# Corleno/Nonstationary_Multivariate_Gaussian_Process

Hardware: AMD Instinct MI355X
Metric: log-posterior evals/sec (N=2048, D=3 nonseparable GP) (higher is better)
Workload: dtype f64

## Files before the change

### nonstationary_multivariate_gaussian_process_amd/csrc/nmgp_api.hip

```cpp
#include <cstdarg>

#include "nmgp_internal.h"

using namespace nmgpk;

enum {
    SC_LOGDET = 0,
    SC_QUAD = 1,
    SC_PRIORQ = 2,
    SC_TRACE = 40,
    SC_OUT = 48,
    SC_MISC = 56,
    SC_COUNT = 128
};

int nmgp_fail(nmgp_ctx* ctx, int code, const char* fmt, ...) {
    char buf[1024];
    va_list ap;
    va_start(ap, fmt);
    vsnprintf(buf, sizeof(buf), fmt, ap);
    va_end(ap);
    if (ctx) ctx->err = buf;
    return code;
}
// ... 122 lines not shown
    c->priors.clear();
}

static void free_subject(nmgp_ctx* c) {
    double** ptrs[] = {&c->d_x, &c->d_Y, &c->d_y, &c->d_pars, &c->d_grad, &c->d_ell, &c->d_sig, &c->d_Lv,
                       &c->d_S, &c->d_Sinv, &c->d_z, &c->d_alpha, &c->d_R, &c->d_R2, &c->d_part, &c->d_K, &c->d_K2,
                       &c->d_w, &c->d_E};
    for (double** p : ptrs) {
        if (*p) hipFree(*p);
        *p = nullptr;
    }
    c->S_cap = c->K_cap = c->part_cap = 0;
    if (c->had_indx) hipFree(c->had_indx);
    if (c->had_y) hipFree(c->had_y);
    c->had_indx = nullptr;
    c->had_y = nullptr;
    c->had = false;
    if (c->ps_buf) hipFree(c->ps_buf);
    c->ps_buf = nullptr;
    c->ps_cap = 0;
    free_priors(c);
    {
        double** bp[] = {&c->b_pars, &c->b_ell, &c->b_Lv, &c->b_S, &c->b_z, &c->b_R, &c->b_scal, &c->b_q,
                         &c->b_S2, &c->b_Sinv, &c->b_alpha, &c->b_part, &c->b_grad, &c->b_R2, &c->b_tr, &c->b_u, &c->b_schur};
        c->b_grad_ready = false;
        c->b_multi = false;
        if (c->b_x) hipFree(c->b_x);
        if (c->b_y) hipFree(c->b_y);
        c->b_x = c->b_y = nullptr;
        for (auto& pf : c->b_priors) {
            if (pf.L) hipFree(pf.L);
            if (pf.logdet) hipFree(pf.logdet);
        }
        c->b_priors.clear();
        for (double** p : bp) {
            if (*p) hipFree(*p);
            *p = nullptr;
        }
        if (c->b_info) hipFree(c->b_info);
        if (c->b_info2) hipFree(c->b_info2);
        c->b_info = c->b_info2 = nullptr;
        c->b_schur_stride = 0;
        c->batch = 0;
    }
}

extern "C" int nmgp_version(void) { return NMGP_VERSION; }

extern "C" int nmgp_device_count(void) {
    int n = 0;
    if (hipGetDeviceCount(&n) != hipSuccess) return 0;
    return n;
}

extern "C" int nmgp_ctx_create(int device, nmgp_ctx** out) {
    if (!out) return NMGP_E_NULL;
    *out = nullptr;
    int ndev = 0;
    if (hipGetDeviceCount(&ndev) != hipSuccess || ndev <= 0) return NMGP_E_HIP;
    if (device < 0 || device >= ndev) return NMGP_E_SHAPE;
    nmgp_ctx* c = new nmgp_ctx();
    c->device = device;
    *out = c;
    if (const char* e = std::getenv("NMGP_CHOL")) c->chol_algo = (std::strcmp(e, "rocsolver") == 0) ? 0 : 1;
    if (const char* e = std::getenv("NMGP_CHOL_NB1")) {
        int v = std::atoi(e);
        if (v >= 64) c->chol_nb1 = (v / 64) * 64;
    }
    HIP_TRY(c, hipSetDevice(device));
    if (const char* e = std::getenv("NMGP_CHOL_LOOKAHEAD")) c->chol_lookahead = std::atoi(e);
    if (const char* e = std::getenv("NMGP_PRIOR_SOLVE")) {
        c->prior_rocblas = std::strcmp(e, "rocblas") == 0;
        c->prior_trsv_all = std::strcmp(e, "trsv") == 0;
    }
    if (const char* e = std::getenv("NMGP_SEP")) c->sep_algo = (std::strcmp(e, "eig") == 0) ? 0 : 1;
    if (const char* e = std::getenv("NMGP_SVC_SCHUR")) c->svc_schur = std::atoi(e) != 0 ? 1 : 0;
    {
        int lo = 0, hi = 0;
        hipDeviceGetStreamPriorityRange(&lo, &hi);
        const bool prio = lo != hi;
        if (prio) HIP_TRY(c, hipStreamCreateWithPriority(&c->stream, hipStreamNonBlocking, hi));
        else HIP_TRY(c, hipStreamCreateWithFlags(&c->stream, hipStreamNonBlocking));
        int la_cus = 64;
        if (const char* e = std::getenv("NMGP_LOOKAHEAD_CUS")) la_cus = std::atoi(e);
        hipDeviceProp_t prop{};
        int ncu = 0;
        if (hipGetDeviceProperties(&prop, device) == hipSuccess) ncu = prop.multiProcessorCount;
        const bool mi355 = std::strncmp(prop.gcnArchName, "gfx950", 6) == 0 && ncu == 256;
        if (mi355 && la_cus > 0 && la_cus < ncu) {
            std::vector<uint32_t> mask((size_t)(ncu + 31) / 32, 0u);
            for (int i = la_cus; i < ncu; ++i) mask[(size_t)i / 32] |= 1u << (i % 32);
            if (hipExtStreamCreateWithCUMask(&c->stream2, (uint32_t)mask.size(), mask.data()) != hipSuccess) {
                (void)hipGetLastError();
                c->stream2 = nullptr;
            } else {
                c->stream2_cus = ncu - la_cus;
            }
        }
        if (!c->stream2) {
// ... 402 lines not shown
                               double* grad) {
    if (!c) return NMGP_E_NULL;
    if (!out5) return nmgp_fail(c, NMGP_E_NULL, "out5 must not be NULL");
    NMGP_TRY(nmgp_svc_set_pars(c, pars));
    NMGP_TRY(svc_enqueue(c, hyper, prior, grad != nullptr));
    return nmgp_svc_fetch(c, out5, grad);
}

static void mass_reset(nmgp_ctx* c) {
    double** ptrs[] = {&c->b_minv, &c->b_vel, &c->b_mchol, &c->b_mU, &c->b_mw, &c->b_mc};
    for (double** p : ptrs) {
        if (*p) hipFree(*p);
        *p = nullptr;
    }
    c->b_mass_kind = 0;
    c->b_mrank = 0;
    c->b_traj_ready = false;
}

static void free_batch(nmgp_ctx* c) {
    double** ptrs[] = {&c->b_pars, &c->b_ell, &c->b_Lv, &c->b_S, &c->b_z, &c->b_R, &c->b_scal, &c->b_q,
                       &c->b_S2, &c->b_Sinv, &c->b_alpha, &c->b_part, &c->b_grad, &c->b_R2, &c->b_tr,
                       &c->b_mom, &c->b_q0, &c->b_g0, &c->b_am, &c->b_av, &c->b_minv, &c->b_vel, &c->b_mchol, &c->b_kin,
                       &c->b_mU, &c->b_mw, &c->b_mc, &c->b_u, &c->b_schur};
    c->b_schur_stride = 0;
    c->b_mass_kind = 0;
    c->b_mrank = 0;
    c->b_cps = 1;
    if (c->b_alive) hipFree(c->b_alive);
    c->b_alive = nullptr;
    c->b_adam_t = -1;
    c->b_grad_ready = false;
    c->b_traj_ready = false;
    if (c->b_hmc) hipFree(c->b_hmc);
    c->b_hmc = nullptr;
    c->b_multi = false;
    if (c->b_x) hipFree(c->b_x);
    if (c->b_y) hipFree(c->b_y);
    c->b_x = c->b_y = nullptr;
    for (auto& pf : c->b_priors) {
        if (pf.L) hipFree(pf.L);
        if (pf.logdet) hipFree(pf.logdet);
    }
    c->b_priors.clear();
    for (double** p : ptrs) {
        if (*p) hipFree(*p);
        *p = nullptr;
    }
// ... 132 lines not shown
    }
    c->b_priors.push_back(pf);
    *out = &c->b_priors.back();
    return 0;
}

static int batch_grad_alloc(nmgp_ctx* c) {
    if (c->b_grad_ready) return 0;
    const size_t N = c->N, T = c->T, n = c->n, P = (size_t)c->P_svc, B = c->batch;
    const size_t ld2 = nmgp_ld(2 * n + 2);
    const size_t NJ = (N + 63) / 64;
    NMGP_TRY(nmgp_dev_alloc(c, &c->b_S2, B * ld2 * n));
    NMGP_TRY(nmgp_dev_alloc(c, &c->b_Sinv, B * n * n));
    NMGP_TRY(nmgp_dev_alloc(c, &c->b_alpha, B * n));
    NMGP_TRY(nmgp_dev_alloc(c, &c->b_part, B * std::max(NJ * N * (T + 1), (size_t)n * ((n + 255) / 256))));
    NMGP_TRY(nmgp_dev_alloc(c, &c->b_grad, B * P));
    NMGP_TRY(nmgp_dev_alloc(c, &c->b_R2, N * B * (1 + T)));
    NMGP_TRY(nmgp_dev_alloc(c, &c->b_tr, B * 2));
    c->b_grad_ready = true;
    return 0;
}

static bool schur_selected(const nmgp_ctx* c, int want_grad) {
    if (want_grad || c->M < 2 || c->svc_schur == 0) return false;
    return true;
}

static int svc_batch_value_schur(nmgp_ctx* c, const double* xs, int xstride, const double* ys, long long ystride, int cps) {
    const int N = c->N, M = c->M, B = c->batch, n1 = (M - 1) * N;
    const long long P = c->P_svc;
    const int xpad = (N + 1) & 1, xoffA = N + 1 + xpad;
    const int ldA = (int)nmgp_ld((size_t)2 * N + 2), ldP = (int)nmgp_ld((size_t)n1 + 1);
    auto r64 = [](size_t v) { return (v + 63) / 64 * 64; };
    const size_t offP = r64((size_t)ldA * N), offPart = r64(offP + (size_t)ldP * n1);
    const size_t need = r64(offPart + (size_t)N * ((N + 255) / 256));
    const size_t bsS = nmgp_ld((size_t)c->n + 1) * (size_t)c->n;
    double* base = c->b_S;
    size_t bsz = bsS;
    if (need > bsS) {
        if (c->b_schur_stride != need) {
            NMGP_TRY(nmgp_dev_alloc(c, &c->b_schur, (size_t)B * need));
            c->b_schur_stride = need;
        }
        base = c->b_schur;
        bsz = need;
    }
    const long long bs = (long long)bsz;
// ... 23 lines not shown
    {
        StageScope sp(c, NMGP_STAGE_REDUCE);
        chol_logdet_quad(s, A, ldA, N, w, c->b_scal + 2, c->b_scal + 3, B, bs, 16);
    }
    {
        StageScope sp(c, NMGP_STAGE_INVERSE);
        const SchurEpi e{xs, c->b_ell, c->b_Lv, tse, ys, c->b_u, Sp, ldP, N, xstride, cps, ystride, bs};
        int r = syrk_schur(s, A + xoffA, ldA, N, M, B, e);
        if (r) return nmgp_fail(c, r, "unsupported number of outputs M=%d", M);
    }
    {
        StageScope sp(c, NMGP_STAGE_CHOL);
        nmgp_potrf(c, Sp, ldP, n1, 1, 0, c->b_info2, B, bs, 1);
    }
    {
        StageScope sp(c, NMGP_STAGE_SOLVE);
        get_row(s, Sp, ldP, n1, w1, n1, B, bs, n1);
    }
    {
        StageScope sp(c, NMGP_STAGE_REDUCE);
        chol_logdet_quad(s, Sp, ldP, n1, w1, c->b_scal + 4, c->b_scal + 5, B, bs, 16);
        svc_schur_combine(s, c->b_Lv, N, M, c->b_scal, 16, c->b_info, c->b_info2, B);
    }
    return 0;
}

extern "C" int nmgp_svc_batch_eval(nmgp_ctx* c, const double hyper[8], int prior, int want_grad) {
    if (!c) return NMGP_E_NULL;
    if (!hyper) return nmgp_fail(c, NMGP_E_NULL, "hyper must not be NULL");
    if (c->batch <= 0) return nmgp_fail(c, NMGP_E_STATE, "nmgp_svc_batch_alloc must be called first");
    HIP_TRY(c, hipSetDevice(c->device));
    const int N = c->N, M = c->M, T = c->T, n = c->n, B = c->batch;
    const long long P = c->P_svc;
    c->b_traj_ready = false;
    if (want_grad) NMGP_TRY(batch_grad_alloc(c));
    const int xpad = (n + 1) & 1, xoff = n + 1 + xpad;
    const int ld = want_grad ? (int)nmgp_ld((size_t)2 * n + 2) : (int)nmgp_ld((size_t)n + 1);
    double* S = want_grad ? c->b_S2 : c->b_S;
    const long long bs = (long long)ld * n;
    const double mu_l = hyper[0], al_l = hyper[1], be_l = hyper[2], mu_L = hyper[3], al_L = hyper[4], be_L = hyper[5];
    const double a = hyper[6], b = hyper[7];
    hipStream_t s = c->stream;
    const bool multi = c->b_multi;
    const int cps = multi ? c->b_cps : 1;
    const double* xs = multi ? c->b_x : c->d_x;
    const int xstride = multi ? N : 0;
    PriorFactor *pl = nullptr, *pL = nullptr;
    if (multi) {
        NMGP_TRY(get_batch_prior(c, al_l, be_l, &pl));
        NMGP_TRY(get_batch_prior(c, al_L, be_L, &pL));
        NMGP_TRY(get_batch_prior(c, al_l, be_l, &pl));
    } else {
        NMGP_TRY(nmgp_get_prior(c, al_l, be_l, &pl));
        NMGP_TRY(nmgp_get_prior(c, al_L, be_L, &pL));
        NMGP_TRY(nmgp_get_prior(c, al_l, be_l, &pl));
    }
    HIP_TRY(c, hipMemsetAsync(c->b_info, 0, (size_t)B * sizeof(int), s));
    if (nmgp_poison()) HIP_TRY(c, hipMemsetAsync(c->b_scal, 0xFF, (size_t)B * 16 * sizeof(double), s));
    PriorStreamScope ps(c);
    if (schur_selected(c, want_grad)) {
        NMGP_TRY(svc_batch_value_schur(c, xs, xstride, multi ? c->b_y : c->d_y, multi ? n : 0, cps));
    } else {
        {
            StageScope sp(c, NMGP_STAGE_COV);
            svc_prep(s, c->b_pars, N, M, c->b_ell, c->b_Lv, B);
            int r = svc_cov_build(s, xs, c->b_ell, c->b_Lv, c->b_pars + (P - 1), S, ld, N, M, false, B, bs, xstride, cps);
            if (r) return nmgp_fail(c, r, "unsupported number of outputs M=%d", M);
        }
        {
            StageScope sp(c, NMGP_STAGE_CHOL);
            set_row(s, S, ld, n, multi ? c->b_y : c->d_y, n, B, bs, multi ? n : 0, cps);
            if (want_grad) identity_rows(s, S, ld, n + 1, n, xpad, B, bs);
            nmgp_potrf(c, S, ld, n, want_grad ? 1 + xpad : 1, want_grad ? n : 0, c->b_info, B, bs, 1);
        }
        {
            StageScope sp(c, NMGP_STAGE_SOLVE);
            get_row(s, S, ld, n, c->b_z, n, B, bs, n);
            if (want_grad) {
                tri_gemv_upper(s, S + xoff, (int)ld, n, c->b_z, c->b_alpha, c->b_part, (int)B, bs,
                               (long long)n * ((n + 255) / 256));
            }
        }
        {
// ... 53 lines not shown
                                          B * (1 + T), &one, pl->L, pl->ld, R, N));
            } else {
                const rocblas_stride sB = (rocblas_stride)(1 + T) * N;
                BLAS_TRY(c, rocblas_dtrsm_strided_batched(ps.hb, rocblas_side_left, rocblas_fill_lower, op,
                                                          rocblas_diagonal_non_unit, N, 1, &one, pl->L, pl->ld, 0, R, N, sB, B));
                BLAS_TRY(c, rocblas_dtrsm_strided_batched(ps.hb, rocblas_side_left, rocblas_fill_lower, op,
                                                          rocblas_diagonal_non_unit, N, T, &one, pL->L, pL->ld, 0, R + N, N, sB,
                                                          B));
            }
            if (pass == 0) col_sumsq(ps.sp, c->b_R, N, N, B * (1 + T), c->b_q);
        }
    }
    ps.done();
    ps.join();
    {
        StageScope sp(c, NMGP_STAGE_REDUCE);
        const double ig_const = a * std::log(b) - std::lgamma(a);
        svc_finalize(s, c->b_scal, c->b_scal + 1, c->b_q, pl->logdet, pL->logdet, c->b_pars, P, N, T, a, b, ig_const,
                     prior, c->b_scal + 8, B, 16, multi ? 1 : 0, cps);
    }
    if (want_grad) {
        {
            StageScope sp(c, NMGP_STAGE_INVERSE);
            syrk_lower(s, S + xoff, ld, c->b_Sinv, n, n, n, n, B, bs, (long long)n * n, 2);
        }
        {
            StageScope sp(c, NMGP_STAGE_ADJOINT);
            trace_terms(s, c->b_alpha, c->b_Sinv, n, n, c->b_tr, -1.0, B);
            int r = svc_adjoint(s, xs, c->b_ell, c->b_Lv, c->b_alpha, c->b_Sinv, n, N, M, c->b_part, -1.0, B, xstride, cps);
            if (r) return nmgp_fail(c, r, "unsupported number of outputs M=%d", M);
            svc_grad_final(s, c->b_part, (N + 63) / 64, N, M, c->b_Lv, c->b_R2, N, c->b_pars, c->b_tr, a, b, prior,
                           c->b_grad, B);
        }
    }
    c->b_last_grad = want_grad != 0;
    c->last_kind = 2;
    return nmgp_take_launch_error(c);
}

extern "C" double* nmgp_svc_batch_grad_dev(nmgp_ctx* c) { return c ? c->b_grad : nullptr; }

extern "C" int nmgp_svc_batch_fetch_grad(nmgp_ctx* c, double* grad) {
    if (!c) return NMGP_E_NULL;
    if (!grad) return nmgp_fail(c, NMGP_E_NULL, "grad must not be NULL");
    if (c->last_kind != 2 || !c->b_last_grad)
        return nmgp_fail(c, NMGP_E_STATE, "the last batched evaluation did not compute gradients");
    HIP_TRY(c, hipSetDevice(c->device));
// ... 717 lines not shown
```

### nonstationary_multivariate_gaussian_process_amd/csrc/nmgp_chol.hip

```cpp
#include "nmgp_internal.h"
#include <cstring>

namespace nmgpk {

static inline int cdiv_c(long long a, long long b) { return (int)((a + b - 1) / b); }

typedef double v4d __attribute__((ext_vector_type(4)));

#define SY_BM 128
#define SY_BK 16
#define SY_LD (SY_BM + 16)
#define SY_SB 8

__device__ __forceinline__ int clamp_row_pair(int r, int rows) {
    int rc = r < rows - 1 ? r : rows - 2;
    return rc < 0 ? 0 : rc;
}

__device__ __forceinline__ double fast_recip(double p) {
    double x = __builtin_amdgcn_rcp(p);
    double e = fma(-p, x, 1.0);
    x = fma(x, e, x);
    e = fma(-p, x, 1.0);
    x = fma(x, e, x);
// ... 160 lines not shown
            const double* __restrict__ Lr = e.Lv + (size_t)r * T_;
            const double xr = e.x[r], lr = e.ell[r];
            const double xr2 = xr * xr, lr2 = lr * lr;
            const double l00 = Lr[0];
            const double il2 = 1.0 / (l00 * l00);
#pragma unroll QU
            for (int q = 0; q < 16; ++q) {
                const int o = 2 * q + hi;
                const int il = pass == 0 ? lo : o, jl = pass == 0 ? o : lo;
                const int c = (pass == 0 ? j0 : i0) + o;
                if (pass == 0 ? (c > r || c >= N) : (c <= r || c >= N)) continue;
                const double* gc = gt + (pass == 0 ? c - col0 : 128 + c - row0) * GS;
                if (pass == 1 && M == 3) {
                    e.S[(size_t)c * e.ld + (Ns + r)] = P[il * 33 + jl];
                    continue;
                }
                const double xc = M <= 4 ? gc[M] : e.x[c], lc = M <= 4 ? gc[M + 1] : e.ell[c];
                const double dist = (xr2 + xc * xc) - 2.0 * (xr * xc);
                const double Aa = lr2 + lc * lc;
                double kv = sqrt(2.0 * (lr * lc) / Aa) * exp(-dist / Aa);
                if (r == c) kv = NMGP_JITTER + kv;
                const double nai = P[il * 33 + jl];
                if (pass == 0) {
                    svc_schur_entries<M, true>(e, sigma2, r, Lr, il2, c, kv, nai, gc);
                    if (M == 3 && c < r) {
                        const double* Lc = e.Lv + (size_t)c * T_;
                        P[il * 33 + jl] = svc_schur_value<M>(sigma2, 2, 1, false, Lc, gc[M - 1], Lr, kv, nai, gt[(128 + r - row0) * GS]);
                    }
                } else {
                    svc_schur_entries<M, false>(e, sigma2, r, Lr, il2, c, kv, nai, gc);
                }
            }
        }
        __builtin_amdgcn_wave_barrier();
    }
}

template <int M>
__device__ __forceinline__ void svc_schur_yrow(const SchurEpi& e, int i) {
    constexpr int T = M * (M + 1) / 2;
    if (i >= e.N) return;
    const size_t Ns = (size_t)e.N;
    const int n1 = (M - 1) * e.N;
    const double sigma2 = exp(e.tse[0]);
    const double* Li = e.Lv + (size_t)i * T;
    const double l00 = Li[0];
// ... 298 lines not shown
            bj = c0 + in / rb;
            bi = base + in % rb;
        }
        }
    }
    if (bi < bj) return;
    bi = __builtin_amdgcn_readfirstlane(bi);
    bj = __builtin_amdgcn_readfirstlane(bj);
    bz = __builtin_amdgcn_readfirstlane(bz);
    A += (size_t)bz * bstride;
    C += (size_t)bz * cstride;
    SchurEpi se{};
    if constexpr (SM > 0) {
        static_assert(NWJ == 4 && BK == 16, "the Schur epilogue assumes 8 waves of 64 x 32");
        constexpr int T = SM * (SM + 1) / 2;
        se = *sep;
        se.x += (size_t)(bz / se.cps) * se.xstride;
        se.y += (size_t)(bz / se.cps) * se.ystride;
        se.ell += (size_t)bz * se.N;
        se.Lv += (size_t)bz * se.N * T;
        se.tse += (size_t)bz * ((size_t)se.N * (1 + T) + 1);
        se.u += (size_t)bz * se.N;
        se.S += (size_t)bz * se.bstride;
    }
    const bool diag = (bi == bj);
    const int tid = threadIdx.x, lane = tid & 63, w = tid >> 6;
    const int wi = w & 1, wj = w >> 1;
    const int row0 = bi * SY_BM, col0 = bj * SY_BM;
    if constexpr (NWJ == 4 && BK == 16) {
        const int ncw = ncols - col0 >= SY_BM ? SY_BM : ncols - col0;
        if (row0 + SY_BM <= mrows && (ncw == SY_BM || ncw == 64) && col0 + SY_BM <= mrows && (K & 31) == 0 &&
            (long long)(K + 16) * lda * 8 < 0x7fff0000LL) {
            int kt0f = ktri ? row0 / BK : 0;
            if (row0 >= tri_row0) {
                const int z = (row0 - tri_row0 - tri_k0) / BK;
                kt0f = z > 0 ? (z & ~1) : 0;
            }
            syrk_tile_fast<SM>(A, lda, C, ldc, K, row0, col0, diag, kt0f, ktri != 0, ncw, yrow, nyr, &sA[0][0], &sB[0][0],
                               skipq && bi == 0 && bj == 0, (finfo != nullptr && bi == 0 && bj == 0) ? finfo + (size_t)bz * fistride : nullptr,
                               fgoff, mirror, fresh0, &se);
            return;
        }
    }
    const int rp = tid & 63, cg = tid >> 6;
    double2 ra[NQ], rb[NQ];

// ... 1404 lines not shown
```

### nonstationary_multivariate_gaussian_process_amd/csrc/nmgp_internal.h

```cpp
#pragma once

#include <hip/hip_runtime.h>
#include <rocblas/rocblas.h>
#include <rocsolver/rocsolver.h>

#include <cmath>
#include <cstdio>
#include <cstdlib>
#include <cstring>
#include <map>
#include <string>
#include <utility>
#include <vector>

#include "nmgp.h"

#define NMGP_JITTER 1e-6
#define NMGP_PRECISION 1e-6

struct DevBuf {
    double* p = nullptr;
    size_t cap = 0;
};

// ... 13 lines not shown
    double bytes = 0;
};

struct SyrkHook {
    void* user = nullptr;
    void* (*begin)(void* user, hipStream_t s, double flop, double bytes) = nullptr;
    void (*end)(void* user, void* token) = nullptr;
};

struct nmgp_ctx {
    int device = 0;
    hipStream_t stream = nullptr;
    hipStream_t stream2 = nullptr;
    int stream2_cus = 0;
    hipStream_t stream_prior = nullptr;
    rocblas_handle blas_prior = nullptr;
    hipEvent_t ev_prior_fork = nullptr, ev_prior_join = nullptr;
    int prior_overlap = 1;
    std::vector<hipEvent_t> chol_ev;
    int chol_lookahead = 1;
    SyrkHook syrk_hook;
    int sep_algo = 1;
    int svc_schur = -1;
    rocblas_handle blas = nullptr;
    std::string err;

    int N = 0, M = 0, T = 0, n = 0;
    double* d_x = nullptr;
    double* d_Y = nullptr;
    double* d_y = nullptr;
    bool had = false;
    int* had_indx = nullptr;
    double* had_y = nullptr;
    long long P_svc = 0;
    double* d_pars = nullptr;
    double* d_grad = nullptr;
    double* d_ell = nullptr;
    double* d_sig = nullptr;
    double* d_Lv = nullptr;
    double* d_S = nullptr;
    double* d_Sinv = nullptr;
    size_t S_cap = 0;
    int ldS = 0;
    double* d_z = nullptr;
    double* d_alpha = nullptr;
    double* d_R = nullptr;
// ... 5 lines not shown
    double* h_pin = nullptr;
    int* h_info = nullptr;
    DevBuf scratch[16];
    std::vector<PriorFactor> priors;
    double* d_K = nullptr;
    double* d_K2 = nullptr;
    size_t K_cap = 0;
    double* d_w = nullptr;
    double* d_E = nullptr;
    int batch = 0;
    double* b_pars = nullptr;
    double* b_ell = nullptr;
    double* b_Lv = nullptr;
    double* b_S = nullptr;
    double* b_z = nullptr;
    double* b_R = nullptr;
    double* b_scal = nullptr;
    double* b_q = nullptr;
    int* b_info = nullptr;
    double* b_u = nullptr;
    int* b_info2 = nullptr;
    double* b_schur = nullptr;
    size_t b_schur_stride = 0;
    bool b_grad_ready = false;
    double* b_S2 = nullptr;
    double* b_Sinv = nullptr;
    double* b_alpha = nullptr;
    double* b_part = nullptr;
    double* b_grad = nullptr;
    double* b_R2 = nullptr;
    double* b_tr = nullptr;
    bool b_last_grad = false;
    double* b_mom = nullptr;
    double* b_q0 = nullptr;
    double* b_g0 = nullptr;
    int* b_hmc = nullptr;
    bool b_traj_ready = false;
    double* b_am = nullptr;
    double* b_av = nullptr;
    int* b_alive = nullptr;
    long long b_adam_t = -1;
    bool b_multi = false;
    double* b_x = nullptr;
    double* b_y = nullptr;
    std::vector<PriorFactor> b_priors;
    int b_cps = 1;
// ... 174 lines not shown
               double b1, double b2, double bc2s, double eps, double step, long long P, int B);
void hmc_status(hipStream_t s, const int* info, const double* scal, int* bad, int* failed, int B);
void hmc_kick_drift(hipStream_t s, double* p, const double* g, double* q, const int* bad, double c, double eps, int drift,
                    long long P, int B);
void hmc_drift(hipStream_t s, double* q, const double* p, const double* vel, const double* minv_diag, double eps, long long P, int B);
void hmc_scale(hipStream_t s, double* p, const double* d, long long P, int B);
void hmc_kinetic(hipStream_t s, const double* p, const double* vel, const double* minv_diag, double* kin, long long P, int B);
void hmc_restore(hipStream_t s, double* q, double* g, const double* q0, const double* g0, int* bad, const int* bad0,
                 const int* accept, long long P, int B);
void prior_trmm(hipStream_t s, bool trans, const double* L0, int ld0, long long s0, const double* L1, int ld1, long long s1,
                const double* in, double* out, int N, int T, long long P, int B, int cps, double coef, int mode, const int* bad);
void prior_trmm_sep(hipStream_t s, bool trans, const double* L0, int ld0, const double* L1, int ld1, const double* in, double* out, int N,
                    int T, long long P, int B, double cscale);
void lowrank_proj(hipStream_t s, const double* U, const double* u, double* c, long long P, int r, int B, int cps);
void lowrank_apply(hipStream_t s, const double* U, const double* wgt, const double* c, const double* in, double* out, long long P,
                   int r, int B, int cps);
void metric_kinetic(hipStream_t s, const double* u, const double* c, const double* sw, double* kin, long long P, int r, int B, int cps);
int svc_adjoint(hipStream_t s, const double* x, const double* ell, const double* Lv, const double* alpha,
                const double* Sinv, int ld, int N, int M, double* part, double ssign = 1.0, int batch = 1,
                int xstride = 0, int cps = 1);
#define NMGP_XTRI_SEED_BLOCKS 3
#define NMGP_TRI_GEMV_BLOCK 256
void tri_gemv_upper(hipStream_t s, const double* W, int ld, int n, const double* z, double* out, double* part, int batch = 1,
                    long long wstride = 0, long long pstride = 0);
void trace_terms(hipStream_t s, const double* alpha, const double* Sinv, int ld, int n, double* out,
                 double ssign = 1.0, int batch = 1);
void svc_grad_final(hipStream_t s, const double* part, int NJ, int N, int M, const double* Lv, const double* R2,
                    int ldR, const double* pars, const double* tr, double a, double b, int prior, double* grad,
                    int batch = 1);
void svc_finalize(hipStream_t s, const double* logdet, const double* quad, const double* q, const double* hl_l,
                  const double* hl_L, const double* pars, long long P, int N, int T, double a, double b,
                  double ig_const, int prior, double* out5, int batch = 1, int sstride = 0, int hstride = 0, int cps = 1);
void half_logdet(hipStream_t s, const double* L, int ld, int n, double* out, int batch = 1);
int kron_mv(hipStream_t s, const double* K, int n1, int n2, const double* y, const double* B, int m1, int m2,
            double* out);
void eig_reduce(hipStream_t s, double* a, const double* wB, int M, const double* wK, int N, const double* sigma2p,
                bool scale, double* out);
void colscale_d(hipStream_t s, const double* V, const double* wB, int M, const double* wK, int N, const double* sigma2p,
                double* Vs);
void colscale(hipStream_t s, const double* V, const double* svec, int rows, int cols, double* Vs);
void sep_coreB(hipStream_t s, const double* At, const double* wB, int M, const double* wK, int N,
               const double* sigma2p, double* coreB);
void sep_adjoint(hipStream_t s, const double* x, const double* ell, const double* sig, const double* U,
                 const double* wB, int M, const double* C, int N, double* part);
void sep_grad_sum(hipStream_t s, const double* part, int NJ, int N, double* g);
void exp_vec(hipStream_t s, const double* in, int n, double* out);
void fill_vec(hipStream_t s, double* out, int n, double v);
// ... 38 lines not shown
                   int small_per, int M, const double* C, int N, double* part, double* g, int B);
void two_col_rhs_b(hipStream_t s, const double* pars, long long P, double mu_a, double mu_b, int N, double* R, int B);
void ps_rows_reduce(hipStream_t s, const double* A, int ld, long long bstride, int n, int R0, int zrow, int E, double* part,
                    int batch, double* dots, double* sqs, long long ostride, long long o0);
void pss_star(hipStream_t s, const double* W0, const double* W1, const double* cv0, const double* cv1, const double* pars, long long P,
              const double* z, int N, int S, double mu_l, double mu_s, double* star, int B);
bool syrk_lower(hipStream_t s, const double* A, int lda, double* C, int ldc, int mrows, int ncols, int K, int batch,
                long long bstride, long long cstride = -1, int ktri = 0, int tri_row0 = 0x7fffffff, int tri_k0 = 0,
                int* finfo = nullptr, int fistride = 0, int goff = 0, const SyrkHook* hook = nullptr);
struct SchurEpi {
    const double* x;
    const double* ell;
    const double* Lv;
    const double* tse;
    const double* y;
    const double* u;
    double* S;
    int ld;
    int N;
    int xstride;
    int cps;
    long long ystride;
    long long bstride;
};
int syrk_schur(hipStream_t s, const double* X, int lda, int N, int M, int batch, const SchurEpi& e);
void identity_rows(hipStream_t s, double* A, int lda, int row0, int n, int pad, int batch = 1, long long bstride = 0);
void set_row(hipStream_t s, double* A, int lda, int row, const double* v, int n, int batch, long long bstride,
             long long vstride, int cps = 1);
void get_row(hipStream_t s, const double* A, int lda, int row, double* v, int n, int batch, long long bstride,
             long long vstride);
void potrf_lower(hipStream_t s, hipStream_t s2, hipEvent_t* ev, double* A, int lda, int n, int extra, int xtri,
                 int nb1, int* info, int batch, long long bstride, int istride, const SyrkHook* hook = nullptr,
                 int precise = 0);

}
```

### nonstationary_multivariate_gaussian_process_amd/csrc/nmgp_kernels.hip

```cpp
#include "nmgp_internal.h"
#include <mutex>

namespace nmgpk {

static inline int cdiv(long long a, long long b) { return (int)((a + b - 1) / b); }

__device__ inline double wave_sum(double v) {
#pragma unroll
    for (int off = 32; off > 0; off >>= 1) v += __shfl_down(v, off, 64);
    return v;
}

__device__ inline double block_sum(double v, double* sh ) {
    int lane = threadIdx.x & 63, w = threadIdx.x >> 6;
    v = wave_sum(v);
    __syncthreads();
    if (lane == 0) sh[w] = v;
    __syncthreads();
    int nw = (blockDim.x + 63) >> 6;
    v = (threadIdx.x < nw) ? sh[threadIdx.x] : 0.0;
    if (w == 0) v = wave_sum(v);
    return v;
}

// ... 223 lines not shown
        default: return NMGP_E_UNSUPPORTED;
    }
    return 0;
}

__global__ __launch_bounds__(256) void k_svc_schur_combine(const double* __restrict__ Lv, int N, int T, double* __restrict__ sc,
                                                            int sstride, int* __restrict__ info, const int* __restrict__ info2) {
    __shared__ double sh[16];
    Lv += (size_t)blockIdx.x * N * T;
    sc += (size_t)blockIdx.x * sstride;
    double a = 0.0;
    for (int i = threadIdx.x; i < N; i += blockDim.x) a += log(Lv[(size_t)i * T]);
    a = block_sum(a, sh);
    if (threadIdx.x == 0) {
        sc[0] = (2.0 * a + sc[2]) + sc[4];
        sc[1] = sc[3] + sc[5];
        if (info[blockIdx.x] == 0 && info2[blockIdx.x] != 0) info[blockIdx.x] = N + info2[blockIdx.x];
    }
}

void svc_schur_combine(hipStream_t s, const double* Lv, int N, int M, double* sc, int sstride, int* info, const int* info2,
                       int batch) {
    NMGP_LAUNCH(k_svc_schur_combine, dim3(batch), dim3(256), 0, s, Lv, N, M * (M + 1) / 2, sc, sstride, info, info2);
}

template <bool GIBBS, bool FULL>
__global__ __launch_bounds__(256) void k_cov_sym(const double* __restrict__ x, const double* __restrict__ sig,
                                                  const double* __restrict__ ell, int N, double alpha, double beta,
                                                  double* __restrict__ out, int ld) {
    constexpr int TJ = 64;
    __shared__ double sx[TJ], sl[TJ], ss[TJ];
    const int I = blockIdx.x, J = blockIdx.y;
    if (!FULL && I < J) return;
    x += (size_t)blockIdx.z * N;
    out += (size_t)blockIdx.z * ld * N;
    const int tid = threadIdx.x, lane = tid & 63, w = tid >> 6;
    const int j0 = J * TJ;
    if (tid < TJ) {
        int j = j0 + tid;
        double xv = (j < N) ? x[j] : 0.0;
        sx[tid] = GIBBS ? xv : xv / beta;
        sl[tid] = (GIBBS && j < N) ? ell[j] : 1.0;
        ss[tid] = (GIBBS && sig != nullptr && j < N) ? sig[j] : 1.0;
    }
    __syncthreads();
    const int i = I * 64 + lane;
// ... 174 lines not shown
    if (i >= n) return;
    const int kn = (n - k0 < 256) ? (n - k0) : 256;
    const double* col = W + i + (size_t)k0 * ld;
    double a0 = 0.0, a1 = 0.0, a2 = 0.0, a3 = 0.0;
    int k = 0;
    for (; k + 8 <= kn; k += 8) {
        const double w0 = col[(size_t)(k + 0) * ld], w1 = col[(size_t)(k + 1) * ld], w2 = col[(size_t)(k + 2) * ld],
                     w3 = col[(size_t)(k + 3) * ld], w4 = col[(size_t)(k + 4) * ld], w5 = col[(size_t)(k + 5) * ld],
                     w6 = col[(size_t)(k + 6) * ld], w7 = col[(size_t)(k + 7) * ld];
        a0 = fma(w0, sz[k + 0], a0);
        a1 = fma(w1, sz[k + 1], a1);
        a2 = fma(w2, sz[k + 2], a2);
        a3 = fma(w3, sz[k + 3], a3);
        a0 = fma(w4, sz[k + 4], a0);
        a1 = fma(w5, sz[k + 5], a1);
        a2 = fma(w6, sz[k + 6], a2);
        a3 = fma(w7, sz[k + 7], a3);
    }
    for (; k < kn; ++k) a0 = fma(col[(size_t)k * ld], sz[k], a0);
    part[(size_t)ch * n + i] = (a0 + a1) + (a2 + a3);
}

__global__ __launch_bounds__(256) void k_tri_gemv_reduce(const double* __restrict__ part, int n, double* __restrict__ out,
                                                          long long pstride) {
    const int i = blockIdx.x * 256 + threadIdx.x;
    if (i >= n) return;
    part += (size_t)blockIdx.y * pstride;
    const int nch = (n + 255) / 256;
    double a = 0.0;
    for (int ch = i / 256; ch < nch; ++ch) a += part[(size_t)ch * n + i];
    out[(size_t)blockIdx.y * n + i] = a;
}

static_assert(NMGP_TRI_GEMV_BLOCK == 256, "k_tri_gemv_part / _reduce are written for 256-wide blocks");
static_assert(NMGP_TRI_GEMV_BLOCK <= 64 * (NMGP_XTRI_SEED_BLOCKS + 1), "tri_gemv_upper would read left of the band k_xtri_seed writes");
void tri_gemv_upper(hipStream_t s, const double* W, int ld, int n, const double* z, double* out, double* part, int batch,
                    long long wstride, long long pstride) {
    const int nb = cdiv(n, 256);
    NMGP_LAUNCH(k_tri_gemv_part, dim3(nb, nb, batch), dim3(256), 0, s, W, ld, n, z, part, wstride, pstride);
    NMGP_LAUNCH(k_tri_gemv_reduce, dim3(nb, batch), dim3(256), 0, s, part, n, out, pstride);
}

__global__ void k_hmc_status(const int* __restrict__ info, const double* __restrict__ scal, int* __restrict__ bad,
                             int* __restrict__ failed, int B) {
    const int z = blockIdx.x * blockDim.x + threadIdx.x;
    if (z >= B) return;
    const double v0 = scal[(size_t)z * 16 + 8], v1 = scal[(size_t)z * 16 + 9];
    const int b = (info[z] != 0 || !isfinite(v0) || !isfinite(v1)) ? 1 : 0;
    bad[z] = b;
    if (failed && b) failed[z] = 1;
}

__global__ __launch_bounds__(256) void k_hmc_kick_drift(double* __restrict__ p, const double* __restrict__ g, double* __restrict__ q,
                                                         const int* __restrict__ bad, double c, double eps, int drift, long long P) {
    const int z = blockIdx.y;
    const long long i = (long long)blockIdx.x * 256 + threadIdx.x;
    if (i >= P) return;
    const size_t o = (size_t)z * P + i;
    double pv = p[o];
    if (!bad[z]) {
        const double t = c * g[o];
        pv = pv - t;
        p[o] = pv;
// ... 581 lines not shown
```

Before: 1693.

## Extend Schur-complement factorization to the gradient path with block inverse assembly

The gradient evaluation now uses the Schur-complement split already used for value-only evaluation: a Cholesky of the N×N block plus a Cholesky of the (M-1)N Schur complement, instead of a full nN Cholesky. The full inverse needed by the adjoint is then assembled blockwise from the small-block inverse, the Schur inverse via syrk, and two batched GEMMs plus custom kernels. The intent is to cut the cubic factorization and inverse cost. The price is extra workspace and more kernel launches, and the gradient path now relies on new, more complex inverse-assembly code. It is on by default.

```diff
diff --git a/nonstationary_multivariate_gaussian_process_amd/csrc/nmgp_api.hip b/nonstationary_multivariate_gaussian_process_amd/csrc/nmgp_api.hip
--- a/nonstationary_multivariate_gaussian_process_amd/csrc/nmgp_api.hip
+++ b/nonstationary_multivariate_gaussian_process_amd/csrc/nmgp_api.hip
@@ -168,7 +168,8 @@
     free_priors(c);
     {
         double** bp[] = {&c->b_pars, &c->b_ell, &c->b_Lv, &c->b_S, &c->b_z, &c->b_R, &c->b_scal, &c->b_q,
-                         &c->b_S2, &c->b_Sinv, &c->b_alpha, &c->b_part, &c->b_grad, &c->b_R2, &c->b_tr, &c->b_u, &c->b_schur};
+                         &c->b_S2, &c->b_Sinv, &c->b_alpha, &c->b_part, &c->b_grad, &c->b_R2, &c->b_tr, &c->b_u, &c->b_schur,
+                         &c->b_schur_g};
         c->b_grad_ready = false;
         c->b_multi = false;
         if (c->b_x) hipFree(c->b_x);
@@ -186,7 +187,7 @@
         if (c->b_info) hipFree(c->b_info);
         if (c->b_info2) hipFree(c->b_info2);
         c->b_info = c->b_info2 = nullptr;
-        c->b_schur_stride = 0;
+        c->b_schur_stride = c->b_schur_g_stride = 0;
         c->batch = 0;
     }
 }
@@ -221,6 +222,7 @@
     }
     if (const char* e = std::getenv("NMGP_SEP")) c->sep_algo = (std::strcmp(e, "eig") == 0) ? 0 : 1;
     if (const char* e = std::getenv("NMGP_SVC_SCHUR")) c->svc_schur = std::atoi(e) != 0 ? 1 : 0;
+    if (const char* e = std::getenv("NMGP_SVC_SCHUR_GRAD")) c->svc_schur_grad = std::atoi(e) != 0 ? 1 : 0;
     {
         int lo = 0, hi = 0;
         hipDeviceGetStreamPriorityRange(&lo, &hi);
@@ -669,8 +671,8 @@
     double** ptrs[] = {&c->b_pars, &c->b_ell, &c->b_Lv, &c->b_S, &c->b_z, &c->b_R, &c->b_scal, &c->b_q,
                        &c->b_S2, &c->b_Sinv, &c->b_alpha, &c->b_part, &c->b_grad, &c->b_R2, &c->b_tr,
                        &c->b_mom, &c->b_q0, &c->b_g0, &c->b_am, &c->b_av, &c->b_minv, &c->b_vel, &c->b_mchol, &c->b_kin,
-                       &c->b_mU, &c->b_mw, &c->b_mc, &c->b_u, &c->b_schur};
-    c->b_schur_stride = 0;
+                       &c->b_mU, &c->b_mw, &c->b_mc, &c->b_u, &c->b_schur, &c->b_schur_g};
+    c->b_schur_stride = c->b_schur_g_stride = 0;
     c->b_mass_kind = 0;
     c->b_mrank = 0;
     c->b_cps = 1;
@@ -849,7 +851,8 @@
 }
 
 static bool schur_selected(const nmgp_ctx* c, int want_grad) {
-    if (want_grad || c->M < 2 || c->svc_schur == 0) return false;
+    if (c->M < 2 || c->svc_schur == 0) return false;
+    if (want_grad) return c->svc_schur_grad != 0;
     return true;
 }
 
@@ -919,6 +922,137 @@
         chol_logdet_quad(s, Sp, ldP, n1, w1, c->b_scal + 4, c->b_scal + 5, B, bs, 16);
         svc_schur_combine(s, c->b_Lv, N, M, c->b_scal, 16, c->b_info, c->b_info2, B);
     }
+    return 0;
+}
+
+struct SchurGrad {
+    double* base;
+    long long bs;
+    int ldA, ldP, ldw, xpadA, xoffA, xpadP, xoffP;
+    size_t offP, offNi, offW, offZp, offTE, offT;
+};
+
+static int schur_grad_layout(nmgp_ctx* c, SchurGrad* g) {
+    const size_t N = c->N, n = c->n, n1 = n - N, B = c->batch;
+    auto r64 = [](size_t v) { return (v + 63) / 64 * 64; };
+    g->xpadA = (int)((N + 1) & 1);
+    g->xoffA = (int)N + 1 + g->xpadA;
+    g->xpadP = (int)((n1 + 1) & 1);
+    g->xoffP = (int)n1 + 1 + g->xpadP;
+    g->ldA = (int)nmgp_ld(2 * N + 2);
+    g->ldP = (int)nmgp_ld(2 * n1 + 2);
+    g->ldw = (int)nmgp_ld(N);
+    const size_t sq = r64((size_t)g->ldw * N);
+    g->offP = r64((size_t)g->ldA * N);
+    g->offNi = r64(g->offP + (size_t)g->ldP * n1);
+    g->offW = g->offNi + sq;
+    g->offZp = g->offW + r64((size_t)g->ldw * n1);
+    g->offTE = g->offZp + sq;
+    g->offT = g->offTE + sq;
+    const size_t need = g->offT + r64(N);
+    const size_t bsS = nmgp_ld(2 * n + 2) * n;
+    if (need <= bsS) {
+        g->base = c->b_S2;
+        g->bs = (long long)bsS;
+        return 0;
+    }
+    if (c->b_schur_g_stride != need) {
+        NMGP_TRY(nmgp_dev_alloc(c, &c->b_schur_g, B * need));
+        c->b_schur_g_stride = need;
+    }
+    g->base = c->b_schur_g;
+    g->bs = (long long)need;
+    return 0;
+}
+
+static int svc_batch_grad_schur(nmgp_ctx* c, const double* xs, int xstride, const double* ys, long long ystride, int cps) {
+    const int N = c->N, M = c->M, n = c->n, B = c->batch, n1 = (M - 1) * N;
+    const long long P = c->P_svc;
+    SchurGrad g;
+    NMGP_TRY(schur_grad_layout(c, &g));
+    const long long bs = g.bs, ps = (long long)n * ((n + 255) / 256);
+    double* A = g.base;
+    double* Sp = g.base + g.offP;
+    double* w = c->b_z;
+    double* w1 = c->b_z + (size_t)B * N;
+    const double* tse = c->b_pars + (P - 1);
+    hipStream_t s = c->stream;
+    HIP_TRY(c, hipMemsetAsync(c->b_info2, 0, (size_t)B * sizeof(int), s));
+    {
+        StageScope sp(c, NMGP_STAGE_COV);
+        svc_prep(s, c->b_pars, N, M, c->b_ell, c->b_Lv, B);
+        int r = svc_schur_a(s, xs, c->b_ell, c->b_Lv, tse, ys, A, g.ldA, g.xpadA, N, M, B, bs, xstride, ystride, cps);
+        if (r) return nmgp_fail(c, r, "unsupported number of outputs M=%d", M);
+    }
+    {
+        StageScope sp(c, NMGP_STAGE_CHOL);
+        nmgp_potrf(c, A, g.ldA, N, 1 + g.xpadA, N, c->b_info, B, bs, 1);
+    }
+    {
+        StageScope sp(c, NMGP_STAGE_SOLVE);
+        get_row(s, A, g.ldA, N, w, N, B, bs, N);
+        tri_gemv_upper(s, A + g.xoffA, g.ldA, N, w, c->b_u, c->b_part, B, bs, ps);
+    }
+    {
+        StageScope sp(c, NMGP_STAGE_REDUCE);
+        chol_logdet_quad(s, A, g.ldA, N, w, c->b_scal + 2, c->b_scal + 3, B, bs, 16);
+    }
+    {
+        StageScope sp(c, NMGP_STAGE_INVERSE);
+        SchurEpi e{xs, c->b_ell, c->b_Lv, tse, ys, c->b_u, Sp, g.ldP, N, xstride, cps, ystride, bs};
+        e.Ai = g.base + g.offNi;
+        e.ldi = g.ldw;
+        int r = syrk_schur(s, A + g.xoffA, g.ldA, N, M, B, e);
+        if (r) return nmgp_fail(c, r, "unsupported number of outputs M=%d", M);
+    }
+    {
+        StageScope sp(c, NMGP_STAGE_CHOL);
+        identity_rows(s, Sp, g.ldP, n1 + 1, n1, g.xpadP, B, bs);
+        nmgp_potrf(c, Sp, g.ldP, n1, 1 + g.xpadP, n1, c->b_info2, B, bs, 1);
+    }
+    {
+        StageScope sp(c, NMGP_STAGE_SOLVE);
+        get_row(s, Sp, g.ldP, n1, w1, n1, B, bs, n1);
+        tri_gemv_upper(s, Sp + g.xoffP, g.ldP, n1, w1, c->b_alpha + N, c->b_part, B, bs, ps, n);
+    }
+    {
+        StageScope sp(c, NMGP_STAGE_REDUCE);
+        chol_logdet_quad(s, Sp, g.ldP, n1, w1, c->b_scal + 4, c->b_scal + 5, B, bs, 16);
+        svc_schur_combine(s, c->b_Lv, N, M, c->b_scal, 16, c->b_info, c->b_info2, B);
+    }
+    return 0;
+}
+
+static int svc_batch_grad_schur_inverse(nmgp_ctx* c) {
+    const int N = c->N, M = c->M, n = c->n, B = c->batch, n1 = (M - 1) * N;
+    const long long P = c->P_svc;
+    SchurGrad g;
+    NMGP_TRY(schur_grad_layout(c, &g));
+    const long long bs = g.bs;
+    double* Ni = g.base + g.offNi;
+    double* W = g.base + g.offW;
+    double* Zp = g.base + g.offZp;
+    double* TE = g.base + g.offTE;
+    const double* tse = c->b_pars + (P - 1);
+    hipStream_t s = c->stream;
+    const double one = 1.0, zero = 0.0;
+    rocblas_atomics_mode am = rocblas_atomics_allowed;
+    BLAS_TRY(c, rocblas_get_atomics_mode(c->blas, &am));
+    BLAS_TRY(c, rocblas_set_atomics_mode(c->blas, rocblas_atomics_not_allowed));
+    syrk_lower(s, g.base + g.offP + g.xoffP, g.ldP, c->b_Sinv + (size_t)N * n + N, n, n1, n1, n1, B, bs, (long long)n * n, 2);
+    sym_mirror_lower(s, Ni, g.ldw, N, B, bs);
+    svc_schur_zw(s, c->b_Lv, tse, c->b_Sinv, W, Zp, g.ldw, N, M, B, bs);
+    rocblas_status st = rocblas_dgemm_strided_batched(c->blas, rocblas_operation_none, rocblas_operation_none, N, n1, N, &one, Ni, g.ldw,
+                                                      bs, W, g.ldw, bs, &one, c->b_Sinv + (size_t)N * n, n, (rocblas_stride)n * n, B);
+    if (st == rocblas_status_success) {
+        svc_schur_tprime(s, c->b_Lv, tse, c->b_Sinv, Zp, TE, g.ldw, N, M, B, bs);
+        st = rocblas_dgemm_strided_batched(c->blas, rocblas_operation_none, rocblas_operation_none, N, N, N, &one, TE, g.ldw, bs, Ni,
+                                           g.ldw, bs, &zero, W, g.ldw, bs, B);
+    }
+    rocblas_set_atomics_mode(c->blas, am);
+    BLAS_TRY(c, st);
+    svc_schur_alpha0(s, c->b_Lv, tse, Ni, g.ldw, c->b_u, c->b_alpha, g.base + g.offT, N, M, B, bs);
+    svc_schur_assemble(s, c->b_Lv, c->b_Sinv, Ni, Zp, W, g.ldw, N, M, B, bs);
     return 0;
 }
 
@@ -955,7 +1089,10 @@
     HIP_TRY(c, hipMemsetAsync(c->b_info, 0, (size_t)B * sizeof(int), s));
     if (nmgp_poison()) HIP_TRY(c, hipMemsetAsync(c->b_scal, 0xFF, (size_t)B * 16 * sizeof(double), s));
     PriorStreamScope ps(c);
-    if (schur_selected(c, want_grad)) {
+    const bool schur = schur_selected(c, want_grad);
+    if (schur && want_grad) {
+        NMGP_TRY(svc_batch_grad_schur(c, xs, xstride, multi ? c->b_y : c->d_y, multi ? n : 0, cps));
+    } else if (schur) {
         NMGP_TRY(svc_batch_value_schur(c, xs, xstride, multi ? c->b_y : c->d_y, multi ? n : 0, cps));
     } else {
         {
@@ -1055,7 +1192,8 @@
     if (want_grad) {
         {
             StageScope sp(c, NMGP_STAGE_INVERSE);
-            syrk_lower(s, S + xoff, ld, c->b_Sinv, n, n, n, n, B, bs, (long long)n * n, 2);
+            if (schur) NMGP_TRY(svc_batch_grad_schur_inverse(c));
+            else syrk_lower(s, S + xoff, ld, c->b_Sinv, n, n, n, n, B, bs, (long long)n * n, 2);
         }
         {
             StageScope sp(c, NMGP_STAGE_ADJOINT);
diff --git a/nonstationary_multivariate_gaussian_process_amd/csrc/nmgp_chol.hip b/nonstationary_multivariate_gaussian_process_amd/csrc/nmgp_chol.hip
--- a/nonstationary_multivariate_gaussian_process_amd/csrc/nmgp_chol.hip
+++ b/nonstationary_multivariate_gaussian_process_amd/csrc/nmgp_chol.hip
@@ -206,6 +206,7 @@
                 if (r == c) kv = NMGP_JITTER + kv;
                 const double nai = P[il * 33 + jl];
                 if (pass == 0) {
+                    if (e.Ai != nullptr) e.Ai[(size_t)c * e.ldi + r] = nai;
                     svc_schur_entries<M, true>(e, sigma2, r, Lr, il2, c, kv, nai, gc);
                     if (M == 3 && c < r) {
                         const double* Lc = e.Lv + (size_t)c * T_;
@@ -550,6 +551,7 @@
         se.tse += (size_t)bz * ((size_t)se.N * (1 + T) + 1);
         se.u += (size_t)bz * se.N;
         se.S += (size_t)bz * se.bstride;
+        if (se.Ai != nullptr) se.Ai += (size_t)bz * se.bstride;
     }
     const bool diag = (bi == bj);
     const int tid = threadIdx.x, lane = tid & 63, w = tid >> 6;
diff --git a/nonstationary_multivariate_gaussian_process_amd/csrc/nmgp_internal.h b/nonstationary_multivariate_gaussian_process_amd/csrc/nmgp_internal.h
--- a/nonstationary_multivariate_gaussian_process_amd/csrc/nmgp_internal.h
+++ b/nonstationary_multivariate_gaussian_process_amd/csrc/nmgp_internal.h
@@ -59,6 +59,7 @@
     SyrkHook syrk_hook;
     int sep_algo = 1;
     int svc_schur = -1;
+    int svc_schur_grad = 1;
     rocblas_handle blas = nullptr;
     std::string err;
 
@@ -110,6 +111,8 @@
     int* b_info2 = nullptr;
     double* b_schur = nullptr;
     size_t b_schur_stride = 0;
+    double* b_schur_g = nullptr;
+    size_t b_schur_g_stride = 0;
     bool b_grad_ready = false;
     double* b_S2 = nullptr;
     double* b_Sinv = nullptr;
@@ -330,7 +333,7 @@
 #define NMGP_XTRI_SEED_BLOCKS 3
 #define NMGP_TRI_GEMV_BLOCK 256
 void tri_gemv_upper(hipStream_t s, const double* W, int ld, int n, const double* z, double* out, double* part, int batch = 1,
-                    long long wstride = 0, long long pstride = 0);
+                    long long wstride = 0, long long pstride = 0, long long ostride = -1);
 void trace_terms(hipStream_t s, const double* alpha, const double* Sinv, int ld, int n, double* out,
                  double ssign = 1.0, int batch = 1);
 void svc_grad_final(hipStream_t s, const double* part, int NJ, int N, int M, const double* Lv, const double* R2,
@@ -415,8 +418,19 @@
     int cps;
     long long ystride;
     long long bstride;
+    double* Ai = nullptr;
+    int ldi = 0;
 };
 int syrk_schur(hipStream_t s, const double* X, int lda, int N, int M, int batch, const SchurEpi& e);
+void sym_mirror_lower(hipStream_t s, double* A, int ld, int n, int batch, long long bstride);
+void svc_schur_zw(hipStream_t s, const double* Lv, const double* tse, double* Sinv, double* W, double* Zp, int ldw, int N, int M,
+                  int batch, long long wstride);
+void svc_schur_tprime(hipStream_t s, const double* Lv, const double* tse, const double* Sinv, double* Zp, double* TE, int ldw, int N,
+                      int M, int batch, long long wstride);
+void svc_schur_alpha0(hipStream_t s, const double* Lv, const double* tse, const double* Ni, int ldw, const double* u, double* alpha,
+                      double* t, int N, int M, int batch, long long wstride);
+void svc_schur_assemble(hipStream_t s, const double* Lv, double* Sinv, const double* Ni, const double* Tp, const double* U, int ldw,
+                        int N, int M, int batch, long long wstride);
 void identity_rows(hipStream_t s, double* A, int lda, int row0, int n, int pad, int batch = 1, long long bstride = 0);
 void set_row(hipStream_t s, double* A, int lda, int row, const double* v, int n, int batch, long long bstride,
              long long vstride, int cps = 1);
diff --git a/nonstationary_multivariate_gaussian_process_amd/csrc/nmgp_kernels.hip b/nonstationary_multivariate_gaussian_process_amd/csrc/nmgp_kernels.hip
--- a/nonstationary_multivariate_gaussian_process_amd/csrc/nmgp_kernels.hip
+++ b/nonstationary_multivariate_gaussian_process_amd/csrc/nmgp_kernels.hip
@@ -269,6 +269,262 @@
 void svc_schur_combine(hipStream_t s, const double* Lv, int N, int M, double* sc, int sstride, int* info, const int* info2,
                        int batch) {
     NMGP_LAUNCH(k_svc_schur_combine, dim3(batch), dim3(256), 0, s, Lv, N, M * (M + 1) / 2, sc, sstride, info, info2);
+}
+
+#define NMGP_SCHUR_MAXB 7
+
+template <int V>
+__device__ __forceinline__ void ld_rows(const double* p, double (&v)[V]) {
+    if constexpr (V == 2) {
+        const double2 t = *reinterpret_cast<const double2*>(p);
+        v[0] = t.x;
+        v[1] = t.y;
+    } else {
+        v[0] = p[0];
+    }
+}
+template <int V>
+__device__ __forceinline__ void st_rows(double* p, const double (&v)[V]) {
+    if constexpr (V == 2) *reinterpret_cast<double2*>(p) = make_double2(v[0], v[1]);
+    else p[0] = v[0];
+}
+
+__global__ __launch_bounds__(256) void k_sym_mirror_lower(double* __restrict__ A, int ld, int n, long long bstride) {
+    __shared__ double t[32][33];
+    const int bi = blockIdx.x, bj = blockIdx.y;
+    if (bi < bj) return;
+    A += (size_t)blockIdx.z * bstride;
+    const int tx = threadIdx.x & 31, ty = threadIdx.x >> 5;
+    const int r0 = bi * 32, c0 = bj * 32;
+#pragma unroll
+    for (int k = 0; k < 4; ++k) {
+        const int c = ty + 8 * k;
+        if (r0 + tx < n && c0 + c < n && r0 + tx >= c0 + c) t[c][tx] = A[(size_t)(c0 + c) * ld + r0 + tx];
+    }
+    __syncthreads();
+#pragma unroll
+    for (int k = 0; k < 4; ++k) {
+        const int r = ty + 8 * k;
+        if (r0 + r < n && c0 + tx < n && r0 + r > c0 + tx) A[(size_t)(r0 + r) * ld + c0 + tx] = t[tx][r];
+    }
+}
+
+void sym_mirror_lower(hipStream_t s, double* A, int ld, int n, int batch, long long bstride) {
+    NMGP_LAUNCH(k_sym_mirror_lower, dim3(cdiv(n, 32), cdiv(n, 32), batch), dim3(256), 0, s, A, ld, n, bstride);
+}
+
+template <int V>
+__global__ __launch_bounds__(256) void k_svc_schur_zw(const double* __restrict__ Lv, const double* __restrict__ tse,
+                                                       double* __restrict__ Sinv, double* __restrict__ W, double* __restrict__ Zp,
+                                                       int ldw, int N, int M, long long wstride) {
+    const int T = M * (M + 1) / 2;
+    const size_t n = (size_t)M * N, Ns = (size_t)N;
+    Lv += (size_t)blockIdx.z * N * T;
+    const double sigma2 = exp(tse[(size_t)blockIdx.z * ((size_t)N * (1 + T) + 1)]);
+    Sinv += (size_t)blockIdx.z * n * n;
+    W += (size_t)blockIdx.z * wstride;
+    Zp += (size_t)blockIdx.z * wstride;
+    const int lane = threadIdx.x & 63, w = threadIdx.x >> 6;
+    const int i = (blockIdx.x * 64 + lane) * V;
+    if (i >= N) return;
+    double lc[V][NMGP_SCHUR_MAXB], Ei[V];
+#pragma unroll
+    for (int h = 0; h < V; ++h) {
+        const double* Li = Lv + (size_t)(i + h) * T;
+        Ei[h] = sigma2 / (Li[0] * Li[0]);
+#pragma unroll
+        for (int c = 1; c <= NMGP_SCHUR_MAXB; ++c) lc[h][c - 1] = c < M ? Li[c * (c + 1) / 2] : 0.0;
+    }
+    for (int k = 0; k < 4; ++k) {
+        const int j = blockIdx.y * 16 + w * 4 + k;
+        if (j >= N) break;
+        double zp[V];
+#pragma unroll
+        for (int h = 0; h < V; ++h) zp[h] = 0.0;
+#pragma unroll
+        for (int b = 1; b <= NMGP_SCHUR_MAXB; ++b) {
+            if (b >= M) break;
+            const double lbj = Lv[(size_t)j * T + b * (b + 1) / 2];
+            double* col = Sinv + ((size_t)b * Ns + j) * n + i;
+            double acc[V], wv[V];
+#pragma unroll
+            for (int h = 0; h < V; ++h) acc[h] = 0.0;
+#pragma unroll
+            for (int c = 1; c <= NMGP_SCHUR_MAXB; ++c) {
+                if (c >= M) break;
+                double r[V];
+                ld_rows<V>(col + (size_t)c * Ns, r);
+#pragma unroll
+                for (int h = 0; h < V; ++h) acc[h] -= lc[h][c - 1] * r[h];
+            }
+#pragma unroll
+            for (int h = 0; h < V; ++h) {
+                wv[h] = Ei[h] * acc[h];
+                zp[h] += acc[h] * lbj;
+            }
+            st_rows<V>(col, acc);
+            st_rows<V>(W + ((size_t)(b - 1) * Ns + j) * ldw + i, wv);
+        }
+        st_rows<V>(Zp + (size_t)j * ldw + i, zp);
+    }
+}
+
+void svc_schur_zw(hipStream_t s, const double* Lv, const double* tse, double* Sinv, double* W, double* Zp, int ldw, int N, int M,
+                  int batch, long long wstride) {
+    if ((N & 1) == 0)
+        NMGP_LAUNCH(k_svc_schur_zw<2>, dim3(cdiv(N, 128), cdiv(N, 16), batch), dim3(256), 0, s, Lv, tse, Sinv, W, Zp, ldw, N, M, wstride);
+    else
+        NMGP_LAUNCH(k_svc_schur_zw<1>, dim3(cdiv(N, 64), cdiv(N, 16), batch), dim3(256), 0, s, Lv, tse, Sinv, W, Zp, ldw, N, M, wstride);
+}
+
+template <int V>
+__global__ __launch_bounds__(256) void k_svc_schur_tprime(const double* __restrict__ Lv, const double* __restrict__ tse,
+                                                           const double* __restrict__ Sinv, double* __restrict__ Zp,
+                                                           double* __restrict__ TE, int ldw, int N, int M, long long wstride) {
+    const int T = M * (M + 1) / 2;
+    const size_t n = (size_t)M * N, Ns = (size_t)N;
+    Lv += (size_t)blockIdx.z * N * T;
+    const double sigma2 = exp(tse[(size_t)blockIdx.z * ((size_t)N * (1 + T) + 1)]);
+    Sinv += (size_t)blockIdx.z * n * n;
+    Zp += (size_t)blockIdx.z * wstride;
+    TE += (size_t)blockIdx.z * wstride;
+    const int lane = threadIdx.x & 63, w = threadIdx.x >> 6;
+    const int i = (blockIdx.x * 64 + lane) * V;
+    if (i >= N) return;
+    for (int k = 0; k < 4; ++k) {
+        const int j = blockIdx.y * 16 + w * 4 + k;
+        if (j >= N) break;
+        const double* Lj = Lv + (size_t)j * T;
+        const double Ej = sigma2 / (Lj[0] * Lj[0]);
+        double gp[V], tp[V], te[V];
+#pragma unroll
+        for (int h = 0; h < V; ++h) gp[h] = 0.0;
+#pragma unroll
+        for (int b = 1; b <= NMGP_SCHUR_MAXB; ++b) {
+            if (b >= M) break;
+            double g[V];
+            ld_rows<V>(Sinv + ((size_t)b * Ns + j) * n + i, g);
+            const double lbj = Lj[b * (b + 1) / 2];
+#pragma unroll
+            for (int h = 0; h < V; ++h) gp[h] += g[h] * lbj;
+        }
+        ld_rows<V>(Zp + (size_t)j * ldw + i, tp);
+#pragma unroll
+        for (int h = 0; h < V; ++h) {
+            tp[h] -= gp[h];
+            te[h] = tp[h] * Ej;
+        }
+        st_rows<V>(Zp + (size_t)j * ldw + i, tp);
+        st_rows<V>(TE + (size_t)j * ldw + i, te);
+    }
+}
+
+void svc_schur_tprime(hipStream_t s, const double* Lv, const double* tse, const double* Sinv, double* Zp, double* TE, int ldw, int N,
+                      int M, int batch, long long wstride) {
+    if ((N & 1) == 0)
+        NMGP_LAUNCH(k_svc_schur_tprime<2>, dim3(cdiv(N, 128), cdiv(N, 16), batch), dim3(256), 0, s, Lv, tse, Sinv, Zp, TE, ldw, N, M, wstride);
+    else
+        NMGP_LAUNCH(k_svc_schur_tprime<1>, dim3(cdiv(N, 64), cdiv(N, 16), batch), dim3(256), 0, s, Lv, tse, Sinv, Zp, TE, ldw, N, M, wstride);
+}
+
+__global__ __launch_bounds__(256) void k_svc_schur_es(const double* __restrict__ Lv, const double* __restrict__ tse,
+                                                       const double* __restrict__ alpha, double* __restrict__ t, int N, int M,
+                                                       long long wstride) {
+    const int T = M * (M + 1) / 2;
+    const int j = blockIdx.x * 256 + threadIdx.x;
+    if (j >= N) return;
+    const double* Lj = Lv + ((size_t)blockIdx.y * N + j) * T;
+    const double sigma2 = exp(tse[(size_t)blockIdx.y * ((size_t)N * (1 + T) + 1)]);
+    alpha += (size_t)blockIdx.y * M * N;
+    double sj = 0.0;
+    for (int b = 1; b < M; ++b) sj += Lj[b * (b + 1) / 2] * alpha[(size_t)b * N + j];
+    t[(size_t)blockIdx.y * wstride + j] = sigma2 / (Lj[0] * Lj[0]) * sj;
+}
+
+__global__ __launch_bounds__(256) void k_svc_schur_alpha0(const double* __restrict__ Lv, const double* __restrict__ Ni, int ldw,
+                                                           const double* __restrict__ u, const double* __restrict__ t,
+                                                           double* __restrict__ alpha, int N, int M, long long wstride) {
+    const int T = M * (M + 1) / 2;
+    const int lane = threadIdx.x & 63;
+    const int i = blockIdx.x * 4 + (threadIdx.x >> 6);
+    if (i >= N) return;
+    const double* col = Ni + (size_t)blockIdx.y * wstride + (size_t)i * ldw;
+    t += (size_t)blockIdx.y * wstride;
+    double a = 0.0;
+    for (int j = lane; j < N; j += 64) a = fma(col[j], t[j], a);
+    a = wave_sum(a);
+    if (lane == 0) {
+        const double* Li = Lv + ((size_t)blockIdx.y * N + i) * T;
+        alpha += (size_t)blockIdx.y * M * N;
+        double si = 0.0;
+        for (int b = 1; b < M; ++b) si += Li[b * (b + 1) / 2] * alpha[(size_t)b * N + i];
+        alpha[i] = ((u[(size_t)blockIdx.y * N + i] - si) - a) / Li[0];
+    }
+}
+
+void svc_schur_alpha0(hipStream_t s, const double* Lv, const double* tse, const double* Ni, int ldw, const double* u, double* alpha,
+                      double* t, int N, int M, int batch, long long wstride) {
+    NMGP_LAUNCH(k_svc_schur_es, dim3(cdiv(N, 256), batch), dim3(256), 0, s, Lv, tse, alpha, t, N, M, wstride);
+    NMGP_LAUNCH(k_svc_schur_alpha0, dim3(cdiv(N, 4), batch), dim3(256), 0, s, Lv, Ni, ldw, u, t, alpha, N, M, wstride);
+}
+
+__global__ __launch_bounds__(256) void k_svc_schur_assemble(const double* __restrict__ Lv, double* __restrict__ Sinv,
+                                                             const double* __restrict__ Ni, const double* __restrict__ Tp,
+                                                             const double* __restrict__ U, int ldw, int N, int M, long long wstride) {
+    __shared__ double ts[32][33], tm[32][33];
+    const int T = M * (M + 1) / 2;
+    const size_t n = (size_t)M * N, Ns = (size_t)N;
+    Lv += (size_t)blockIdx.z * N * T;
+    Sinv += (size_t)blockIdx.z * n * n;
+    Ni += (size_t)blockIdx.z * wstride;
+    Tp += (size_t)blockIdx.z * wstride;
+    U += (size_t)blockIdx.z * wstride;
+    const int tx = threadIdx.x & 31, ty = threadIdx.x >> 5;
+    const int i0 = blockIdx.x * 32, j0 = blockIdx.y * 32;
+    const int i = i0 + tx;
+#pragma unroll
+    for (int k = 0; k < 4; ++k) {
+        const int c = ty + 8 * k;
+        if (j0 + tx < N && i0 + c < N) ts[c][tx] = Tp[(size_t)(i0 + c) * ldw + j0 + tx];
+    }
+    const double di = i < N ? Lv[(size_t)i * T] : 1.0;
+    double gp[4] = {0.0, 0.0, 0.0, 0.0};
+    for (int b = 1; b < M; ++b) {
+#pragma unroll
+        for (int k = 0; k < 4; ++k) {
+            const int jl = ty + 8 * k, j = j0 + jl;
+            if (i < N && j < N) {
+                double* p = Sinv + ((size_t)b * Ns + j) * n + i;
+                const double g = *p;
+                gp[k] += g * Lv[(size_t)j * T + b * (b + 1) / 2];
+                const double o = g / di;
+                *p = o;
+                tm[jl][tx] = o;
+            }
+        }
+        __syncthreads();
+#pragma unroll
+        for (int k = 0; k < 4; ++k) {
+            const int r = ty + 8 * k;
+            if (i0 + r < N && j0 + tx < N) Sinv[(size_t)(i0 + r) * n + (size_t)b * Ns + j0 + tx] = tm[tx][r];
+        }
+        __syncthreads();
+    }
+    if (M < 2) __syncthreads();
+#pragma unroll
+    for (int k = 0; k < 4; ++k) {
+        const int jl = ty + 8 * k, j = j0 + jl;
+        if (i < N && j < N) {
+            const double dj = Lv[(size_t)j * T];
+            const double v = ((Ni[(size_t)j * ldw + i] - gp[k]) + ts[tx][jl]) + U[(size_t)j * ldw + i];
+            Sinv[(size_t)j * n + i] = v / (di * dj);
+        }
+    }
+}
+
+void svc_schur_assemble(hipStream_t s, const double* Lv, double* Sinv, const double* Ni, const double* Tp, const double* U, int ldw,
+                        int N, int M, int batch, long long wstride) {
+    NMGP_LAUNCH(k_svc_schur_assemble, dim3(cdiv(N, 32), cdiv(N, 32), batch), dim3(256), 0, s, Lv, Sinv, Ni, Tp, U, ldw, N, M, wstride);
 }
 
 template <bool GIBBS, bool FULL>
@@ -489,23 +745,23 @@
 }
 
 __global__ __launch_bounds__(256) void k_tri_gemv_reduce(const double* __restrict__ part, int n, double* __restrict__ out,
-                                                          long long pstride) {
+                                                          long long pstride, long long ostride) {
     const int i = blockIdx.x * 256 + threadIdx.x;
     if (i >= n) return;
     part += (size_t)blockIdx.y * pstride;
     const int nch = (n + 255) / 256;
     double a = 0.0;
     for (int ch = i / 256; ch < nch; ++ch) a += part[(size_t)ch * n + i];
-    out[(size_t)blockIdx.y * n + i] = a;
+    out[(size_t)blockIdx.y * ostride + i] = a;
 }
 
 static_assert(NMGP_TRI_GEMV_BLOCK == 256, "k_tri_gemv_part / _reduce are written for 256-wide blocks");
 static_assert(NMGP_TRI_GEMV_BLOCK <= 64 * (NMGP_XTRI_SEED_BLOCKS + 1), "tri_gemv_upper would read left of the band k_xtri_seed writes");
 void tri_gemv_upper(hipStream_t s, const double* W, int ld, int n, const double* z, double* out, double* part, int batch,
-                    long long wstride, long long pstride) {
+                    long long wstride, long long pstride, long long ostride) {
     const int nb = cdiv(n, 256);
     NMGP_LAUNCH(k_tri_gemv_part, dim3(nb, nb, batch), dim3(256), 0, s, W, ld, n, z, part, wstride, pstride);
-    NMGP_LAUNCH(k_tri_gemv_reduce, dim3(nb, batch), dim3(256), 0, s, part, n, out, pstride);
+    NMGP_LAUNCH(k_tri_gemv_reduce, dim3(nb, batch), dim3(256), 0, s, part, n, out, pstride, ostride < 0 ? (long long)n : ostride);
 }
 
 __global__ void k_hmc_status(const int* __restrict__ info, const double* __restrict__ scal, int* __restrict__ bad,
```

Result: no change. 1682 (-0.6%).
